# UT-Austin-RPL/FORGE

Measured on AMD Instinct MI355X. Metric: rendered views/sec (5 views, 128^2 px, 64^3 voxel), higher is better.
Workload: dtype f32; 1 GPU; BASELINE configs[1]: FORGE hot path, 1 scene(s)/GPU x 5 input views 256^2 -> 32^3x128 feature grid -> 64^3 render grid -> 5 views x 128^2 rays x 64 samples -> 5 RGB 256^2; HIP rotate, fp32-MFMA implicit-GEMM ResNet-50 trunk / conv1 / ConvGRU (Winograd F(2x2,3x3) x 3 depth taps) / heads / conv_rgb, HIP ray-march (no MIOpen/rocBLAS kernel in the step); eval BN, random-init seeded weights; scenes_per_gpu=1, views_in=5, views_out=5, feature_grid=32, render_grid=64, steps_in_flight=4, launch=hipGraph replay, 4 steps in flight on 4 HIP streams, parallelism=dp1 (scene-sharded, no data-path collective; 4-scalar RCC...

## Files before the change

forge_amd/_lib.py:

```python
import ctypes
import os

import torch

_HERE = os.path.dirname(os.path.abspath(__file__))
LIB_PATH = os.environ.get("FORGE_AMD_LIB") or os.path.join(_HERE, "libforge_hip.so")
_lib = None

_P = ctypes.c_void_p
_I = ctypes.c_int
_F = ctypes.c_float
_D = ctypes.c_double
_LL = ctypes.c_longlong

SIGNATURES = {
    "forge_version": [],
    "forge_last_error": [],
    "forge_rotate_fwd": [_P, _P, _P, _P, _I, _I, _I, _I, _I, _P],
    "forge_rotate_fwd_slots": [_P, _P, _P, _P, _P, _I, _I, _I, _I, _I, _P],
    "forge_rotate_xf_from_poses": [_P, _P, _P, _P, _P, _I, _I, _F, _P],
    "forge_rotate_bwd": [_P, _P, _P, _P, _P, _P, _I, _I, _I, _I, _I, _P],
    "forge_pose_chain_fwd": [_P, _P, _P, _P, _P, _F, _I, _I, _P, _P, _P, _P, _P, _P, _P, _P],
    "forge_colsum": [_P, _I, _P, _P, _LL, _I, _P],
    "forge_adam_small": [_P, _P, _P, _P, _P, _I, _F, _F, _F, _F, _P],
# ... 7 lines not shown
    "forge_resize_bilinear_bwd": [_P, _P, _I, _I, _I, _I, _I, _P],
    "forge_conv_igemm": [_P, _I, _I, _LL, _P, _I, _I, _LL, _P, _P, _P, _P, _F, _P, _P, _P, _P, _P, _P] + [_I] * 10 + [_P] + [_I] * 12 + [_P, _LL, _P, _P],
    "forge_wino_weights": [_P, _P, _I, _I, _I, _I, _P],
    "forge_wino_dy": [_P, _I, _P, _I, _I, _I, _I, _I, _P],
    "forge_wino_wgrad": [_P, _P, _I, _LL, _LL, _P, _I, _LL, _LL, _P, _I, _I, _I, _I, _I, _I, _P],
    "forge_wino_dw": [_P, _P, _I, _I, _I, _P],
    "forge_wino_input": [_P, _I, _LL, _P, _I, _LL, _I, _I, _I, _I, _I, _I, _LL, _P],
    "forge_wino_input_dy": [_P, _I, _P, _P, _I, _I, _I, _I, _I, _P],
    "forge_wino_gemm": [_P, _I, _I, _LL, _LL, _P, _I, _I, _LL, _LL, _P, _P, _I, _I, _I, _I, _I, _I, _I, _P],
    "forge_wino_gemm_half": [_P, _I, _I, _LL, _LL, _P, _I, _I, _LL, _LL, _P, _P, _I, _I, _I, _I, _I, _I, _P],
    "forge_wino_gemm_dn": [_P, _I, _I, _LL, _LL, _P, _I, _I, _LL, _LL, _P, _P, _I, _I, _I, _I, _I, _I, _P],
    "forge_wino_weights_dn": [_P, _P, _I, _I, _P],
    "forge_wino_input_dn4": [_P, _I, _LL, _P, _I, _LL, _I, _I, _I, _I, _I, _I, _LL, _P],
    "forge_wino_weights_dn4": [_P, _P, _I, _I, _P],
    "forge_wino_gemm_dn4": [_P, _I, _I, _LL, _LL, _P, _I, _I, _LL, _LL, _P, _P, _I, _I, _I, _I, _I, _I, _P],
    "forge_wino_input_dn4h": [_P, _I, _LL, _P, _I, _LL, _I, _I, _I, _I, _I, _I, _LL, _P],
    "forge_wino_weights_dn4h": [_P, _P, _I, _I, _P],
    "forge_wino_gemm_dn4h": [_P, _I, _I, _LL, _LL, _P, _I, _I, _LL, _LL, _P, _P, _I, _I, _I, _I, _I, _I, _P],
    "forge_wino_output_dn4h": [_P, _P, _P, _P, _P, _P, _P, _P, _P, _I, _I, _I, _I, _I, _I, _I, _P],
    "forge_wino_output_half": [_P, _P, _LL, _LL, _P, _P, _P, _F, _P, _P, _P, _P, _P, _P, _I, _I, _I, _I, _I, _I, _I, _P],
    "forge_wino_gemm_tile": [_LL, _I, _I],
    "forge_wino_output": [_P, _P, _LL, _LL, _P, _P, _P, _F, _P, _P, _P, _P, _P, _P, _I, _I, _I, _I, _I, _I, _I, _P],
    "forge_conv_igemm_plan": [_LL, _I, _I, _I, _I, _I, _I, _LL, _P, _P],
    "forge_conv_wgrad": [_P, _I, _P, _I, _I, _LL, _P, _I, _I, _LL, _P] + [_I] * 9 + [_P, _I, _P],
    "forge_conv_direct_fwd": [_P, _I, _P, _P, _F, _P, _I] + [_I] * 6 + [_P, _I, _P],
    "forge_conv_direct_dgrad": [_P, _I, _P, _P, _I] + [_I] * 6 + [_P, _I, _P],
    "forge_conv_direct_wgrad": [_P, _I, _P, _I, _P] + [_I] * 6 + [_P, _I, _P],
    "forge_gru_gates_fwd": [_P, _P, _P, _P, _P, _LL, _I, _P],
    "forge_gru_state_fwd": [_P, _P, _P, _P, _LL, _I, _P],
    "forge_gru_state_bwd": [_P, _I, _P, _P, _P, _P, _P, _P, _LL, _I, _P, _LL, _LL, _I, _P],
    "forge_gru_gates_bwd": [_P, _P, _I, _P, _P, _P, _P, _P, _P, _I, _LL, _I, _P, _LL, _LL, _I, _P],
    "forge_bn_ws_doubles": [_I],
    "forge_bn_train_fwd": [_P, _I, _P, _P, _F, _F, _P, _I, _P, _P, _P, _P, _F, _P, _LL, _I, _P, _I, _P, _I, _P],
    "forge_bn_train_bwd": [_P, _I, _P, _I, _P, _P, _P, _P, _F, _P, _I, _P, _P, _P, _LL, _I, _P, _I, _P, _I, _P],
    "forge_bn_sync_stats": [_P, _I, _P, _LL, _I, _I, _P],
    "forge_bn_eval_fwd": [_P, _I, _P, _P, _P, _P, _F, _F, _P, _I, _P, _P, _LL, _I, _P, _I, _P],
    "forge_bn_sync_fwd_apply": [_P, _I, _P, _P, _F, _F, _P, _I, _P, _P, _P, _P, _F, _P, _LL, _LL, _I, _P, _I, _P, _P],
    "forge_bn_sync_bwd_reduce": [_P, _I, _P, _I, _P, _P, _P, _P, _F, _P, _P, _P, _LL, _I, _P, _I, _P],
    "forge_bn_sync_bwd_apply": [_P, _I, _P, _I, _P, _P, _P, _P, _F, _P, _I, _P, _LL, _LL, _I, _P, _I, _P, _I, _P],
    "forge_affine_act_bwd": [_P, _I, _P, _I, _P, _F, _P, _I, _LL, _I, _P],
    "forge_sse_groups_blocks": [],
    "forge_sse_groups_fwd": [_P, _LL, _LL, _LL, _LL, _P, _P] + [_I] * 7 + [_P],
    "forge_sse_groups_bwd": [_P, _LL, _LL, _LL, _LL, _P, _P, _P] + [_I] * 7 + [_P],
    "forge_attention_fwd": [_P, _P, _P, _LL, _P, _I, _I, _I, _I, _P],
    "forge_attention_fwd_lse": [_P, _P, _P, _LL, _P, _P, _I, _I, _I, _I, _P],
    "forge_attention_bwd": [_P, _P, _P, _LL, _P, _P, _P, _P, _P, _P, _P, _I, _I, _I, _I, _P],
# ... 94 lines not shown
```

forge_amd/convops.py:

```python
import collections
import ctypes
import functools
import os
from fractions import Fraction

import torch

from . import _lib, determinism

EPI_BIAS, EPI_AFFINE_ACT, EPI_GRU_GATES, EPI_GRU_OUT = 0, 1, 2, 3


_TAPS_CACHE = {}


def _taps_array(taps):
    key = tuple(tuple(t) for t in taps)
    arr = _TAPS_CACHE.get(key)
    if arr is None:
        flat = [int(v) for t in key for v in t]
        arr = _TAPS_CACHE[key] = (ctypes.c_int * len(flat))(*flat)
    return arr


# ... 154 lines not shown

GRAD_ZEROS = _ZeroArena()


def grad_zeros(shape, device, scratch=False):
    if scratch:
        return torch.zeros(tuple(shape), dtype=torch.float32, device=device)
    return GRAD_ZEROS.zeros(tuple(shape), device)


SPLITK_WS_BYTES = 128 << 20

TILE_NAMES = {"A": "128, 128, 8, 1", "B": "64, 128, 8, 1", "C": "128, 64, 8, 1", "D": "64, 64, 4, 1", "E": "128, 32, 4, 1"}

_PLAN_CACHE = {}


class _State:
    plan_override = None
    winograd = True
    wino_depth_nest = os.environ.get("FORGE_WINO_DEPTH_NEST", "1") != "0"
    wino_depth_nest4 = os.environ.get("FORGE_WINO_DEPTH_NEST4", "1") != "0"
    wino_h4 = os.environ.get("FORGE_WINO_H4", "1") != "0"


STATE = _State()


class force_plan:

    def __init__(self, tile=None, ksplit=None):
        self.val = (tile, ksplit)

    def __enter__(self):
        self.prev = STATE.plan_override
        STATE.plan_override = self.val
        return self

    def __exit__(self, *exc):
        STATE.plan_override = self.prev
        return False


def conv_plan(M, Cout, Cin, ntaps, epilogue, ldo, nphase=1):
    key = (int(M), int(Cout), int(Cin), int(ntaps), int(nphase), int(epilogue), int(ldo) % 4 == 0)
    pl = _PLAN_CACHE.get(key)
    if pl is None:
        tile, ks = ctypes.c_int(0), ctypes.c_int(0)
        _lib.check(_lib.lib().forge_conv_igemm_plan(int(M), int(Cout), int(Cin), int(ntaps), int(nphase), int(epilogue), int(ldo), SPLITK_WS_BYTES,
                                                    ctypes.byref(tile), ctypes.byref(ks)), "forge_conv_igemm_plan")
        pl = _PLAN_CACHE[key] = (chr(tile.value), ks.value)
    ov = STATE.plan_override
    if ov is not None and pl[0] != "N":
        tile = ov[0] or pl[0]
        ks = ov[1] if ov[1] is not None else (pl[1] if ov[0] is None else 1)
        can_split = nphase == 1 and epilogue in (EPI_BIAS, EPI_AFFINE_ACT) and Cout % 4 == 0 and ldo % 4 == 0
        if ks > 1 and not (can_split and ks * M * Cout * 4 <= SPLITK_WS_BYTES and ks <= (ntaps // nphase) * (Cin // 32)):
            ks = 1
        return tile, ks
    return pl


MAX_OPERAND_BYTES = (1 << 31) - 1


@_lib.on_tensor_device
def conv_igemm(in1, C1, ld1, in2, C2, ld2, wp, bias, scale, shift, slope, residual, aux_h, aux_z, out, out2,
               grid, in_grid, Cout, ldo, taps, out_grid=None, istride=1, ostride=1, phase=(0, 0, 0), epilogue=EPI_BIAS,
               bs1=0, bs2=0, lift=0, out3=None, stats=None):
    n, D, H, W = grid
    Di, Hi, Wi = in_grid
    Do, Ho, Wo = out_grid if out_grid is not None else (D, H, W)
    if wp.shape != (len(taps), Cout, C1 + C2):
        raise ValueError("packed weight %s does not match taps=%d Cout=%d Cin=%d" % (tuple(wp.shape), len(taps), Cout, C1 + C2))
    in_rows, out_rows = Di * Hi * Wi, Do * Ho * Wo
    b1, b2 = (int(bs1) or in_rows), (int(bs2) or in_rows)
    span = lambda k, br, ld: ((k - 1) * br + in_rows) * ld * 4
    limit = MAX_OPERAND_BYTES
    nc = n
    while nc > 1 and (span(nc, b1, ld1) > limit or (in2 is not None and span(nc, b2, ld2) > limit)):
        nc = (nc + 1) // 2
    L, st, arr = _lib.lib(), _lib.current_stream(), _taps_array(taps)
    nphase = 1
    if tuple(phase) == (-1, -1, -1):
        nphase = 8 if Do == 2 * D else 4

    def off(t, floats):
        return None if t is None else ctypes.c_void_p(t.data_ptr() + 4 * floats)
    gate_w = Cout // 2 if epilogue == EPI_GRU_GATES else Cout
    for s0 in range(0, n, nc):
        k = min(nc, n - s0)
        orow = s0 * out_rows
        tile, ksplit = conv_plan(k * D * H * W, Cout, C1 + C2, len(taps), epilogue, ldo, nphase)
        if stats is not None and (ksplit > 1 or nc < n):
            raise RuntimeError("forge_amd: conv_igemm output statistics need an un-chunked launch without split-K (use conv_stats_buffer)")
        ws = torch.empty(ksplit * k * D * H * W * Cout, dtype=torch.float32, device=out.device) if ksplit > 1 else None
        o_ld = gate_w if epilogue == EPI_GRU_GATES else ldo
        _lib.check(L.forge_conv_igemm(
            off(in1, s0 * b1 * ld1), C1, ld1, int(bs1), off(in2, s0 * b2 * ld2), C2, ld2, int(bs2), _lib.ptr(wp), _lib.ptr(bias), _lib.ptr(scale),
            _lib.ptr(shift), float(slope), off(residual, orow * (Cout if (lift or epilogue in (EPI_GRU_GATES, EPI_GRU_OUT)) else ldo)),
            off(aux_h, orow * gate_w), off(aux_z, orow * Cout),
            off(out, orow * (Cout if lift else o_ld)), off(out2, orow * o_ld), off(out3, orow * o_ld), k, D, H, W, istride, Di, Hi, Wi, Cout, ldo,
            arr, len(taps), ostride, phase[0], phase[1], phase[2], Do, Ho, Wo, epilogue, int(lift), 0 if tile == "N" else ord(tile), ksplit,
            _lib.ptr(ws), 0 if ws is None else ws.numel() * 4, _lib.ptr(stats), st),
            "forge_conv_igemm")
# ... 226 lines not shown
        Mm = torch.empty(P, R, Cout, dtype=torch.float32, device=device)
    if not (Mm.is_contiguous() and Mm.dtype == torch.float32 and Mm.numel() >= P * R * Cout):
        raise ValueError("point-product buffer %s %s%s cannot hold %d x %d x %d float32" % (
            tuple(Mm.shape), Mm.dtype, "" if Mm.is_contiguous() else " (not contiguous)", P, R, Cout))
    if Mm.shape != (P, R, Cout):
        Mm = Mm.as_strided((P, R, Cout), (R * Cout, Cout, 1))
    return Mm


@_lib.on_tensor_device
def wino_form_gemm(form, V1, C1, V2, C2, U, Mm, n, D, Ht, Wt, Cout, view=0, views=1):
    R = n * D * Ht * Wt
    vol = int(D * Ht * Wt * form.rows)
    nest = form.kloops is not None
    kd = 3 if nest else U.shape[1]
    if U.shape != form.ushape(kd, Cout, C1 + C2) or (kd not in (1, 3)) or (nest and not U.is_contiguous()):
        raise ValueError("%s weight %s does not match Cout=%d Cin=%d" % ("depth-nest" if nest else "transformed", tuple(U.shape), Cout, C1 + C2))
    if form.rows != 1 and (V1.shape[1] != n * views * vol or (V2 is not None and V2.shape[1] != n * vol)):
        raise ValueError("depth-nest operands %s / %s are not %s's %d (x %d views) rows per point" % (
            tuple(V1.shape), None if V2 is None else tuple(V2.shape), form.input, n * vol, views))
    Mm = _point_products(Mm, form.P, R, Cout, V1.device)
    tile = (ord(wino_gemm_tile(R, Cout, C1 + C2)),) if form.tile else ()
    p1 = ctypes.c_void_p(V1.data_ptr() + 4 * view * vol * C1)
    _lib.check(getattr(_lib.lib(), form.gemm)(p1, C1, C1, views * vol if views > 1 else 0, V1.shape[1] * C1, _lib.ptr(V2), C2, C2, 0,
                                              0 if V2 is None else V2.shape[1] * C2, _lib.ptr(U), _lib.ptr(Mm), n, D, Ht, Wt, Cout, kd,
                                              *tile, _lib.current_stream()), form.gemm)
    return Mm


def wino_gemm(V1, C1, V2, C2, U, Mm, n, D, Ht, Wt, Cout, view=0, views=1, half=None):
    if U.dim() == 5:
        form = "dn"
    else:
        if half is None:
            half = WINO_FORMS["half"].applies(n * D * Ht * Wt, D, Ht, Wt, Cout, C1 + C2)
        form = "half" if half else "points"
    return wino_form_gemm(WINO_FORMS[form], V1, C1, V2, C2, U, Mm, n, D, Ht, Wt, Cout, view=view, views=views)


def wino_gemm_tile(R, Cout, Cin):
    ov = STATE.plan_override
    if ov is not None and ov[0]:
        return ov[0]
    return chr(_lib.lib().forge_wino_gemm_tile(int(R), int(Cout), int(Cin)))


@_lib.on_tensor_device
def wino_output(Mm, bias, scale, shift, slope, residual, aux_h, aux_z, out, out2, out3, n, D, H, W, Cout, ldo, epilogue, Mm2=None, view=0, views=1):
    P = Mm.shape[0] if Mm.dim() == 3 else 0
# ... 401 lines not shown
```

forge_amd/csrc/conv_igemm.hip:

```cpp
#include "common.h"
#include <cmath>
#include <type_traits>

namespace forge {

enum ConvEpilogue : int {
    EPI_BIAS = 0,
    EPI_AFFINE_ACT = 1,
    EPI_GRU_GATES = 2,
    EPI_GRU_OUT = 3,
};

constexpr int MAX_TAPS = 64;

struct ConvArgs {
    const float* in1; const float* in2;
    int C1, C2, ld1, ld2;
    long long bs1r, bs2r;
    long long span1, span2;
    const float* wp;
    const float* bias;
    const float* scale; const float* shift; float slope;
    const float* aux_h; const float* aux_z;
    float* out; float* out2; float* out3;
    int n, D, H, W;
    int is, Di, Hi, Wi;
    const float* residual; int ldr;
    int Cout, ldo;
    int ntaps;
    int os, pz, py, px, Do, Ho, Wo;
    int nphase, tpp;
    int epi;
    int lift;
    int nbat;
    long long pt1, pt2, ptw, pto;
    float* ws; int ksplit;
    double* stats;
    signed char tap[MAX_TAPS][4];
};

constexpr int BK = 32, NTHREADS = 512;
constexpr int RS_STAGES = 2;

#ifdef FORGE_CONV_TIMING
__device__ long long g_conv_stamp[8192 * 4];
#define FORGE_STAMP(k) do { if (threadIdx.x == 0 && blockIdx.x < 8192) g_conv_stamp[blockIdx.x * 4 + (k)] = wall_clock64(); } while (0)
extern "C" int forge_debug_conv_stamps(long long* host, int n) {
    return (int)hipMemcpyFromSymbol(host, HIP_SYMBOL(g_conv_stamp), (size_t)n * 4 * sizeof(long long));
}
#else
#define FORGE_STAMP(k) do { } while (0)
#endif

__device__ __forceinline__ int lds_off(int row, int chunk) {
    return row * BK + ((chunk ^ ((row >> 1) & 7)) << 2);
}

struct LanePos { int wm, wn, half, l31; };

struct ReadA {
// ... 71 lines not shown
        store(1, [&](int r) { return acc[1][0][0][r] - acc[0][0][0][r]; });
        FORGE_STAMP(3);
    }
}

template <int BM, int BN, int NW, int MT = 1, int RS = 0>
__global__ __launch_bounds__(NW * 64) void conv_igemm_kernel(const ConvArgs a) {
    constexpr int NP = RS ? 4 : 1;
    constexpr int WM = BM / (32 * MT), WN = NW / WM;
    constexpr int NT = BN / (32 * WN);
    static_assert(NT >= 1 && WM * WN == NW && NT * 32 * WN == BN && WM * 32 * MT == BM, "unsupported tile");
    constexpr int A_FLOATS = BM * BK, B_FLOATS = BN * BK;
    constexpr int RPP = NW * 8;
    constexpr int ACH = BM / RPP, BCH = BN / RPP;
    static_assert(ACH >= 1 && BCH >= 1, "tile too small for the workgroup");
    extern __shared__ __attribute__((aligned(16))) float smem[];

    FORGE_STAMP(0);
    const int tid = threadIdx.x, lane = tid & 63, wave = tid >> 6;
    const int wm = wave / WN, wn = wave % WN;
    const long long M = (long long)a.n * a.D * a.H * a.W;
    const int ntile_n = (a.Cout + BN - 1) / BN;
    const unsigned bid_all = xcd_remap(blockIdx.x, gridDim.x);
    const int ks = (int)(bid_all % (unsigned)a.ksplit);
    unsigned bid = bid_all / (unsigned)a.ksplit;
    int phase = 0;
    if (a.nphase > 1) {
        phase = (int)(bid % (unsigned)a.nphase);
        bid /= (unsigned)a.nphase;
    }
    const int pz = a.nphase > 1 ? (a.nphase == 8 ? (phase >> 2) & 1 : 0) : a.pz;
    const int py = a.nphase > 1 ? (phase >> 1) & 1 : a.py, px = a.nphase > 1 ? phase & 1 : a.px;
    const int t_lo = phase * a.tpp;
    constexpr int PLANES = RS == 2 ? 2 : RS == 3 ? 4 : 1;
    long long pb = 0;
    if (a.nbat > 1) {
        const unsigned tiles = (PLANES > 1 ? (unsigned)(M / (PLANES * BM)) : (unsigned)((M + BM - 1) / BM)) * (unsigned)ntile_n;
        pb = bid / tiles;
        bid -= (unsigned)pb * tiles;
    }
    float* const outp = a.out + pb * a.pto;
    const long long m0 = [&]() -> long long {
        if constexpr (PLANES > 1) {
            const unsigned tpl = (unsigned)(a.H * a.W) / BM;
            const unsigned ti = bid / ntile_n, grp = ti / tpl;
            return (long long)((unsigned)PLANES * grp * tpl + (ti - grp * tpl)) * BM;
        } else {
            return (long long)(bid / ntile_n) * BM;
        }
    }();
    const int n0 = (bid % ntile_n) * BN;
    const int Cin = a.C1 + a.C2;
    const int kchunks = Cin / BK;
    const int nsteps_all = a.tpp * kchunks;
    const int s_begin = (int)((long long)ks * nsteps_all / a.ksplit), s_end = (int)((long long)(ks + 1) * nsteps_all / a.ksplit);
    const int nsteps = s_end - s_begin;

    forge_v4i32 w1 = make_rsrc_words(a.in1 + pb * a.pt1, a.span1), w2 = make_rsrc_words(a.in2 ? a.in2 + pb * a.pt2 : a.in1, a.in2 ? a.span2 : 0),
                ww = make_rsrc_words(a.wp + pb * a.ptw, (long long)a.ntaps * a.Cout * Cin * 4);
    const unsigned lds_wave = lds_addr(smem) + (unsigned)__builtin_amdgcn_readfirstlane(wave) * 1024u;
    const int cp = tid & 7;
    int ar[ACH], az[ACH], ay[ACH], ax[ACH], an[ACH], asrc[ACH];
    bool aval[ACH];
#pragma unroll
    for (int j = 0; j < ACH; ++j) {
        ar[j] = (tid >> 3) + RPP * j;
        const long long vl = m0 + ar[j];
        aval[j] = vl < M;
        unsigned v = aval[j] ? (unsigned)vl : 0u;
        unsigned q = v / (unsigned)a.W;
        ax[j] = (int)(v - q * (unsigned)a.W) * a.is; v = q;
        q = v / (unsigned)a.H;
        ay[j] = (int)(v - q * (unsigned)a.H) * a.is; v = q;
        q = v / (unsigned)a.D;
        az[j] = (int)(v - q * (unsigned)a.D) * a.is;
        an[j] = (int)q;
        asrc[j] = (cp ^ ((ar[j] >> 1) & 7)) << 2;
    }
    int br[BCH]; unsigned boff[BCH];
#pragma unroll
    for (int j = 0; j < BCH; ++j) {
        br[j] = (tid >> 3) + RPP * j;
        const int bsrc = (cp ^ ((br[j] >> 1) & 7)) << 2;
        boff[j] = (n0 + br[j]) < a.Cout ? (unsigned)(((n0 + br[j]) * Cin + bsrc) * 4) : OOB;
    }

    constexpr bool KC_OUTER = (BM == 128 && BN == 128);
    static_assert(!RS || (!KC_OUTER && MT == 1), "the row-stage form exists on the tap-outer tiles");
    __shared__ int sdelta[KC_OUTER ? 2 * MAX_TAPS : 1];
    unsigned long long vmask[KC_OUTER ? ACH : 1];
    unsigned base1[KC_OUTER ? ACH : 1], base2[KC_OUTER ? ACH : 1];
    if constexpr (KC_OUTER) {
#pragma unroll
        for (int j = 0; j < ACH; ++j) {
            const int sp = (az[j] * a.Hi + ay[j]) * a.Wi + ax[j];
            base1[j] = (unsigned)(((an[j] * (int)a.bs1r + sp) * a.ld1 + asrc[j]) * 4);
            base2[j] = (unsigned)(((an[j] * (int)a.bs2r + sp) * a.ld2 + asrc[j]) * 4);
            vmask[j] = 0ull;
        }
        for (int tt = 0; tt < a.ntaps; ++tt) {
            const int dz = a.tap[tt][0], dy = a.tap[tt][1], dx = a.tap[tt][2];
#pragma unroll
            for (int j = 0; j < ACH; ++j) {
                const int zi = az[j] + dz, yi = ay[j] + dy, xi = ax[j] + dx;
                const bool ok = aval[j] && (unsigned)zi < (unsigned)a.Di && (unsigned)yi < (unsigned)a.Hi && (unsigned)xi < (unsigned)a.Wi;
                vmask[j] |= (unsigned long long)ok << tt;
            }
        }
        if (tid < a.ntaps) {
            const int d = (a.tap[tid][0] * a.Hi + a.tap[tid][1]) * a.Wi + a.tap[tid][2];
            sdelta[tid] = d * a.ld1 * 4;
            sdelta[MAX_TAPS + tid] = d * a.ld2 * 4;
        }
        __syncthreads();
    }
    unsigned eoff[ACH], eoff2[ACH];
    auto prep_tap = [&](int t) {
        if constexpr (KC_OUTER) {
            const unsigned d1 = (unsigned)sdelta[t], d2 = (unsigned)sdelta[MAX_TAPS + t];
#pragma unroll
            for (int j = 0; j < ACH; ++j) {
                const bool ok = (vmask[j] >> t) & 1ull;
                eoff[j] = ok ? base1[j] + d1 : OOB;
                eoff2[j] = ok ? base2[j] + d2 : OOB;
            }
        } else {
            const int dz = a.tap[t][0], dy = a.tap[t][1], dx = a.tap[t][2];
#pragma unroll
            for (int j = 0; j < ACH; ++j) {
                const int zi = az[j] + dz, yi = ay[j] + dy, xi = ax[j] + dx;
                const bool ok = aval[j] && (unsigned)zi < (unsigned)a.Di && (unsigned)yi < (unsigned)a.Hi && (unsigned)xi < (unsigned)a.Wi;
                const int sp = (zi * a.Hi + yi) * a.Wi + xi;
                eoff[j] = ok ? (unsigned)(((an[j] * (int)a.bs1r + sp) * a.ld1 + asrc[j]) * 4) : OOB;
                eoff2[j] = ok ? (unsigned)(((an[j] * (int)a.bs2r + sp) * a.ld2 + asrc[j]) * 4) : OOB;
            }
        }
    };
    auto issue_step = [&](int t, int kc, int buf) {
        const int c0 = kc * BK;
        const unsigned stage = lds_wave + (unsigned)buf * (unsigned)((A_FLOATS + B_FLOATS) * 4);
        if (c0 < a.C1) {
#pragma unroll
            for (int j = 0; j < ACH; ++j) lds_dma16(w1, eoff[j] + (unsigned)(c0 * 4), stage + (unsigned)(j * NW * 1024));
        } else {
#pragma unroll
            for (int j = 0; j < ACH; ++j) lds_dma16(w2, eoff2[j] + (unsigned)((c0 - a.C1) * 4), stage + (unsigned)(j * NW * 1024));
        }
        const unsigned wbase = (unsigned)((t * a.Cout * Cin + c0) * 4);
#pragma unroll
        for (int j = 0; j < BCH; ++j) lds_dma16(ww, boff[j] + wbase, stage + (unsigned)(A_FLOATS * 4 + j * NW * 1024));
    };
    constexpr int NACC = RS == 3 ? 4 : RS ? 3 : 1;
    f32x16 accs[NACC][MT][NT];
#pragma unroll
    for (int q = 0; q < NACC; ++q)
#pragma unroll
        for (int i = 0; i < MT; ++i)
#pragma unroll
            for (int j = 0; j < NT; ++j)
#pragma unroll
                for (int r = 0; r < 16; ++r) accs[q][i][j][r] = 0.f;
    f32x16 (&acc)[MT][NT] = accs[0];

    const int half = lane >> 5, l31 = lane & 31;
    int kc, t;
    if constexpr (KC_OUTER) { kc = s_begin / a.tpp; t = s_begin - kc * a.tpp; }
    else { t = s_begin / kchunks; kc = s_begin - t * kchunks; }
    t += t_lo;
    auto advance = [&]() {
        if constexpr (KC_OUTER) {
            if (++t == t_lo + a.tpp) { t = t_lo; ++kc; }
            prep_tap(t);
        } else {
            if (++kc == kchunks) { kc = 0; ++t; prep_tap(t); }
        }
    };
    if constexpr (!RS) {
        prep_tap(t);
        issue_step(t, kc, 0);
        lds_dma_wait();
        __syncthreads();
        FORGE_STAMP(1);
    }
    const LanePos lp{wm, wn, half, l31};
    [[maybe_unused]] const unsigned HW = (unsigned)(a.H * a.W);
    [[maybe_unused]] const int col0 = n0 + wn * (BN / WN);
    if constexpr (!RS) {
    int buf = 0;
#pragma unroll
    for (int q = 0; q < NP; ++q) {
        for (int s = 0; s < nsteps; ++s) {
            const float* sa = smem + buf * (A_FLOATS + B_FLOATS);
            const float* sb = sa + A_FLOATS;
            if (s + 1 < nsteps) {
                advance();
                issue_step(t, kc, buf ^ 1);
            }
#pragma unroll
            for (int g = 0; g < 4; ++g) mfma_group<BN, WN, MT, NT>(lp, accs[q], sa, sb, g, ReadA{});
            lds_dma_wait();
            __syncthreads();
            buf ^= 1;
// ... 134 lines not shown
                }
            } else if (q == 3) {
#pragma unroll
                for (int r = 0; r < 16; ++r) {
                    const float S = accs[2][0][0][r] + accs[3][0][0][r], Dl = accs[2][0][0][r] - accs[3][0][0][r];
                    accs[2][0][0][r] = fmaf(4.f, S, accs[0][0][0][r]);
                    accs[3][0][0][r] = fmaf(2.f, Dl, accs[1][0][0][r]);
                    accs[0][0][0][r] = accs[0][0][0][r] + S;
                    accs[1][0][0][r] = fmaf(8.f, Dl, accs[1][0][0][r]);
                }
                store(1, accs[3][0][0]);
                store(2, accs[2][0][0]);
            } else if (q == 4) {
                store(0, accs[0][0][0]);
            }
        }
        FORGE_STAMP(2);
        store(3, accs[1][0][0]);
        FORGE_STAMP(3);
    }
    if constexpr (RS != 0) return;

    FORGE_STAMP(2);
    const int Ch = a.Cout / 2;
    const bool remap = (a.os != 1) || (a.Do != a.D) || (a.Ho != a.H) || (a.Wo != a.W);
    long long* s_row = reinterpret_cast<long long*>(smem);
    if (a.ksplit == 1 && tid < BM) {
        const long long m = m0 + tid;
        long long o = -1;
        if (m < M) {
            if (a.lift > 0) {
                const unsigned HW = (unsigned)(a.H * a.W), nn = (unsigned)m / HW, hw = (unsigned)m - nn * HW;
                o = ((long long)nn * a.lift * HW + hw) * (a.Cout / a.lift);
            } else if (remap) {
                unsigned q = (unsigned)m, t2 = q / (unsigned)a.W;
                const int x = (int)(q - t2 * (unsigned)a.W); q = t2; t2 = q / (unsigned)a.H;
                const int y = (int)(q - t2 * (unsigned)a.H); q = t2; t2 = q / (unsigned)a.D;
                const int z = (int)(q - t2 * (unsigned)a.D);
                o = (((long long)t2 * a.Do + (z * a.os + pz)) * a.Ho + (y * a.os + py)) * a.Wo + (x * a.os + px);
            } else {
                o = m;
            }
        }
        s_row[tid] = o;
    }
    __syncthreads();
// ... 454 lines not shown
                ++rounds;
            }
            const double traffic_us = ((double)M * K * 4.0 * ntn + (double)Cout * K * 4.0 + (double)M * Cout * 4.0) / 4.0e6;
            if (us < traffic_us) us = traffic_us;
            us += (double)(rounds + 1) * t.ov * sqrt((double)t.bm * t.bn / 16384.0);
            if (k > 1) us += 3.0 + (double)(k + 1) * M * Cout * 4.0 / 2.0e6;
            if (us < best_us) { best_us = us; best = ConvPlan{t.id, k}; }
        }
    }
    return best;
}

template <int RS>
static int launch_point_form(const ConvArgs& a, int planes, size_t lds, const char* entry, hipStream_t st) {
    const long long M = (long long)a.n * a.D * a.H * a.W;
    const long long grid = ((M + 64 * planes - 1) / (64 * planes)) * ((a.Cout + 127) / 128) * a.nbat;
    FORGE_REQUIRE(grid < (1ll << 31), FORGE_ESHAPE, "%s: grid too large", entry);
    FORGE_REQUIRE(RS != 1 || M * a.ldo * 4 < (1ll << 31), FORGE_ESHAPE, "%s: an output plane spans >= 2 GiB (32-bit buffer offsets); split the batch", entry);
    FORGE_SET_MAX_LDS_ONCE((conv_igemm_kernel<64, 128, 8, 1, RS>), lds);
    hipLaunchKernelGGL((conv_igemm_kernel<64, 128, 8, 1, RS>), dim3((unsigned)grid), dim3(8 * 64), lds, st, a);
    return 0;
}

static int launch_conv_tile(const ConvArgs& a, char tile, hipStream_t st, int row_stage = 0) {
    const long long M = (long long)a.n * a.D * a.H * a.W;
    auto nblk = [&](int bm, int bn) { return ((M + bm - 1) / bm) * ((a.Cout + bn - 1) / bn); };
    if (row_stage == 1) { const size_t lds = RS_STAGES * (64 * BK + 128 * BK) * sizeof(float); return launch_point_form<1>(a, 1, lds, "forge_wino_gemm_half", st); }
    if (row_stage == 2) { const size_t lds = RS_STAGES * (2 * 64 * BK + 128 * BK) * sizeof(float); return launch_point_form<2>(a, 2, lds, "forge_wino_gemm_dn", st); }
    if (row_stage == 3) { const size_t lds = RS_STAGES * (64 * BK + 128 * BK) * sizeof(float); return launch_point_form<3>(a, 4, lds, "forge_wino_gemm_dn4", st); }
#define FORGE_LAUNCH_CONV(BMv, BNv, NWv)                                                                                   \
    do {                                                                                                                   \
        const long long grid = nblk(BMv, BNv) * a.ksplit * a.nphase * a.nbat;                                              \
        FORGE_REQUIRE(grid < (1ll << 31), FORGE_ESHAPE, "forge_conv_igemm: grid too large");                                \
        const size_t lds = 2 * (BMv * BK + BNv * BK) * sizeof(float);                                                      \
        FORGE_SET_MAX_LDS_ONCE((conv_igemm_kernel<BMv, BNv, NWv>), lds);                                                   \
        hipLaunchKernelGGL((conv_igemm_kernel<BMv, BNv, NWv>), dim3((unsigned)grid), dim3(NWv * 64), lds, st, a);          \
    } while (0)
    switch (tile) {
        case 'A': FORGE_LAUNCH_CONV(128, 128, 8); break;
        case 'B': FORGE_LAUNCH_CONV(64, 128, 8); break;
        case 'C': FORGE_LAUNCH_CONV(128, 64, 8); break;
        case 'E': FORGE_LAUNCH_CONV(128, 32, 4); break;
        default: FORGE_LAUNCH_CONV(64, 64, 4); break;
    }
#undef FORGE_LAUNCH_CONV
    return 0;
}

}

using namespace forge;

extern "C" int forge_conv_igemm_plan(long long M, int Cout, int Cin, int ntaps, int nphase, int epilogue, int ldo, long long splitk_ws_bytes,
                                     int* tile, int* ksplit) {
    FORGE_REQUIRE(tile && ksplit && M > 0 && Cout > 0 && Cin > 0 && ntaps > 0 && (nphase == 1 || nphase == 4 || nphase == 8) && ntaps % nphase == 0,
                  FORGE_EINVAL, "forge_conv_igemm_plan: bad argument");
    if (Cout <= 16) { *tile = 'N'; *ksplit = 1; return 0; }
    const ConvPlan pl = plan_conv(M * nphase, Cout, Cin, ntaps / nphase,
                                  nphase == 1 && splitk_ws_bytes > 0 && (epilogue == EPI_BIAS || epilogue == EPI_AFFINE_ACT) && Cout % 4 == 0 && ldo % 4 == 0,
                                  splitk_ws_bytes);
    *tile = pl.tile; *ksplit = pl.ksplit;
    return 0;
}

extern "C" int forge_conv_igemm(const float* in1, int C1, int ld1, long long bs1, const float* in2, int C2, int ld2, long long bs2,
                                const float* wp,
                                const float* bias, const float* scale, const float* shift, float slope, const float* residual,
                                const float* aux_h, const float* aux_z, float* out, float* out2, float* out3,
                                int n, int D, int H, int W, int is, int Di, int Hi, int Wi, int Cout, int ldo,
                                const int* taps, int ntaps, int os, int pz, int py, int px, int Do, int Ho, int Wo,
                                int epilogue, int lift, int tile, int ksplit, float* splitk_ws, long long splitk_ws_bytes, double* stats,
                                forge_stream_t stream) {
    FORGE_REQUIRE(in1 && wp && out && taps, FORGE_EINVAL, "forge_conv_igemm: null pointer argument");
    FORGE_REQUIRE(stats == nullptr || (epilogue == EPI_BIAS && ksplit <= 1 && Cout > 16 && !(pz < 0) && lift == 0), FORGE_EINVAL,
                  "forge_conv_igemm: output statistics need the plain bias epilogue of the wide kernel without split-K, phases or lift");
    FORGE_REQUIRE(n > 0 && D > 0 && H > 0 && W > 0 && Cout > 0 && ntaps > 0 && ntaps <= MAX_TAPS, FORGE_EINVAL,
                  "forge_conv_igemm: bad dims n=%d D=%d H=%d W=%d Cout=%d ntaps=%d", n, D, H, W, Cout, ntaps);
    const int kstep = Cout <= 16 ? 16 : 32;
    FORGE_REQUIRE(C1 > 0 && C1 % kstep == 0 && C2 >= 0 && C2 % kstep == 0, FORGE_ESHAPE,
                  "forge_conv_igemm: C1=%d / C2=%d must be multiples of the K-step %d (16 for Cout <= 16, else 32)", C1, C2, kstep);
    FORGE_REQUIRE((C2 == 0) == (in2 == nullptr), FORGE_EINVAL, "forge_conv_igemm: in2/C2 mismatch");
    FORGE_REQUIRE(epilogue >= 0 && epilogue <= 3, FORGE_EINVAL, "forge_conv_igemm: unknown epilogue %d", epilogue);
    FORGE_REQUIRE(epilogue != EPI_AFFINE_ACT || (scale && shift), FORGE_EINVAL, "forge_conv_igemm: affine epilogue needs scale/shift");
    FORGE_REQUIRE(epilogue != EPI_GRU_GATES || (aux_h && out2 && Cout % 2 == 0), FORGE_EINVAL, "forge_conv_igemm: GRU gate epilogue needs aux_h, out2");
    FORGE_REQUIRE(epilogue != EPI_GRU_OUT || (aux_h && aux_z), FORGE_EINVAL, "forge_conv_igemm: GRU out epilogue needs aux_h, aux_z");
    FORGE_REQUIRE(os >= 1 && Do > 0 && Ho > 0 && Wo > 0, FORGE_EINVAL, "forge_conv_igemm: bad output mapping");
    FORGE_REQUIRE(is >= 1 && Di > 0 && Hi > 0 && Wi > 0, FORGE_EINVAL, "forge_conv_igemm: bad input mapping");
    FORGE_REQUIRE(lift == 0 || (lift > 0 && epilogue == EPI_AFFINE_ACT && Cout % lift == 0 && D == 1 && os == 1 && Cout > 64), FORGE_EINVAL,
                  "forge_conv_igemm: lift needs the affine epilogue on a 2-D (D=1) conv with Cout %% lift == 0 and Cout > 64");
    FORGE_REQUIRE(ld1 >= C1 && ld1 % 4 == 0 && (C2 == 0 || (ld2 >= C2 && ld2 % 4 == 0)) && ldo >= 1, FORGE_EINVAL,
                  "forge_conv_igemm: row strides must cover the channels and keep 16-byte alignment");
    ConvArgs a;
    a.in1 = in1; a.in2 = in2; a.C1 = C1; a.C2 = C2; a.ld1 = ld1; a.ld2 = ld2;
    a.bs1r = bs1 > 0 ? bs1 : (long long)Di * Hi * Wi; a.bs2r = bs2 > 0 ? bs2 : (long long)Di * Hi * Wi;
    a.span1 = ((long long)(n - 1) * a.bs1r + (long long)Di * Hi * Wi) * ld1 * 4;
    a.span2 = in2 ? ((long long)(n - 1) * a.bs2r + (long long)Di * Hi * Wi) * ld2 * 4 : 0;
    FORGE_REQUIRE(a.span1 < (1ll << 31) && a.span2 < (1ll << 31) && (long long)ntaps * Cout * (C1 + C2) * 4 < (1ll << 31), FORGE_ESHAPE,
                  "forge_conv_igemm: an operand spans >= 2 GiB (32-bit buffer offsets); split the batch");
    a.is = is; a.Di = Di; a.Hi = Hi; a.Wi = Wi; a.residual = residual;
    a.ldr = (lift > 0 || epilogue == EPI_GRU_GATES || epilogue == EPI_GRU_OUT) ? Cout : ldo;
    a.lift = lift; a.ws = nullptr; a.ksplit = 1; a.stats = stats;
    a.wp = wp; a.bias = bias; a.scale = scale; a.shift = shift; a.slope = slope;
    a.aux_h = aux_h; a.aux_z = aux_z; a.out = out; a.out2 = out2; a.out3 = out3; a.n = n; a.D = D; a.H = H; a.W = W; a.Cout = Cout; a.ldo = ldo;
    a.ntaps = ntaps; a.os = os; a.pz = pz; a.py = py; a.px = px; a.Do = Do; a.Ho = Ho; a.Wo = Wo; a.epi = epilogue;
    a.nphase = 1; a.tpp = ntaps; a.nbat = 1; a.pt1 = a.pt2 = a.ptw = a.pto = 0;
    if (pz < 0) {
        FORGE_REQUIRE(os == 2 && py < 0 && px < 0 && Ho == 2 * H && Wo == 2 * W && (Do == 2 * D || Do == D), FORGE_EINVAL,
                      "forge_conv_igemm: merged phases (pz = py = px = -1) need os = 2 and a doubled output grid");
        a.nphase = Do == 2 * D ? 8 : 4;
        FORGE_REQUIRE(ntaps % a.nphase == 0, FORGE_EINVAL, "forge_conv_igemm: merged phases need ntaps %% %d == 0", a.nphase);
        a.tpp = ntaps / a.nphase;
        a.pz = a.py = a.px = 0;
    }
    for (int k = 0; k < 3 * ntaps; ++k)
        FORGE_REQUIRE(taps[k] >= -128 && taps[k] <= 127, FORGE_EINVAL, "forge_conv_igemm: tap %d component %d = %d outside [-128, 127]", k / 3, k % 3, taps[k]);
    for (int t = 0; t < MAX_TAPS; ++t) {
        for (int k = 0; k < 3; ++k) a.tap[t][k] = (signed char)(t < ntaps ? taps[t * 3 + k] : 0);
        a.tap[t][3] = 0;
    }
    const long long M = (long long)n * D * H * W;
    FORGE_REQUIRE(M < (1ll << 31), FORGE_ESHAPE, "forge_conv_igemm: more than 2^31 GEMM rows; split the batch");
    FORGE_REQUIRE(out3 == nullptr || epilogue == EPI_GRU_GATES || epilogue == EPI_GRU_OUT, FORGE_EINVAL, "forge_conv_igemm: out3 is a GRU-epilogue output");
    hipStream_t st = (hipStream_t)stream;
    if (Cout <= 16) {
// ... 121 lines not shown
```

include/forge_hip.h:

```cpp
#ifndef FORGE_HIP_H
#define FORGE_HIP_H

#ifdef __cplusplus
extern "C" {
#endif

typedef void* forge_stream_t;

#define FORGE_EINVAL (-1)
#define FORGE_ESHAPE (-2)

int forge_version(void);
const char* forge_last_error(void);

int forge_rotate_fwd(const float* vox, const float* xf, const int* mode, float* out,
                     int n, int C, int D, int H, int W, forge_stream_t stream);

int forge_rotate_fwd_slots(const float* vox, const float* xf, const int* mode, const int* dst_slot, float* out,
                           int n, int C, int D, int H, int W, forge_stream_t stream);

int forge_rotate_xf_from_poses(const float* poses, float* xf, int* mode, int* slot, const float* dist, int B, int t, float half_extent,
                               forge_stream_t stream);

int forge_pose_chain_fwd(const float* rot, const float* trans, const float* can_pose, const float* can_extr, const float* K, float half_extent,
// ... 16 lines not shown
                       const float* K, long long k0, long long k1, long long k2, float* cam16, float* origin, int V, forge_stream_t stream);

long long forge_render_bwd_ws_bytes(int V, int C, int Hr, int Wr, int S, int want_cam);
int forge_render_bwd(const float* feat, const float* dens, const float* cam, const int* view2vol,
                     const float* g_feat, const float* g_opac, const float* g_depth,
                     float* dfeat, float* ddens, float* dcam,
                     int V, int nvol, int C, int D, int H, int W, int Hr, int Wr, int S,
                     float zmin, float zmax, float hx, float hy, float hz,
                     void* ws, long long ws_bytes, forge_stream_t stream);

int forge_resize_bilinear_fwd(const float* in, float* out, int P, int Hi, int Wi, int Ho, int Wo, forge_stream_t stream);
int forge_resize_bilinear_bwd(const float* g, float* din, int P, int Hi, int Wi, int Ho, int Wo, forge_stream_t stream);

int forge_conv_igemm(const float* in1, int C1, int ld1, long long bs1, const float* in2, int C2, int ld2, long long bs2,
                     const float* wp,
                     const float* bias, const float* scale, const float* shift, float slope, const float* residual,
                     const float* aux_h, const float* aux_z, float* out, float* out2, float* out3,
                     int n, int D, int H, int W, int is, int Di, int Hi, int Wi, int Cout, int ldo,
                     const int* taps, int ntaps, int os, int pz, int py, int px, int Do, int Ho, int Wo,
                     int epilogue, int lift, int tile, int ksplit, float* splitk_ws, long long splitk_ws_bytes, double* stats, forge_stream_t stream);

int forge_conv_igemm_plan(long long M, int Cout, int Cin, int ntaps, int nphase, int epilogue, int ldo, long long splitk_ws_bytes,
                          int* tile, int* ksplit);

int forge_wino_weights(const float* wp, float* U, int Cout, int Cin, int kd, int transpose, forge_stream_t stream);
int forge_wino_dy(const float* dy, int ldy, float* dM, int n, int D, int H, int W, int Cout, forge_stream_t stream);
int forge_wino_wgrad(const float* dMm, const float* V1, int C1, long long bs1, long long pt1, const float* V2, int C2, long long bs2,
                     long long pt2, float* dU, int n, int D, int Ht, int Wt, int Cout, int kd, forge_stream_t stream);
int forge_wino_dw(const float* dU, float* dw, int Cout, int Cin, int kd, forge_stream_t stream);
int forge_wino_input(const float* in, int ld, long long bs, float* V, int ldv, long long ptv, int n, int D, int H, int W, int C,
                     int nsum , long long sum_stride,
                     forge_stream_t stream);
int forge_wino_input_dy(const float* dy, int ld, float* V, float* dM, int n, int D, int H, int W, int C, forge_stream_t stream);
int forge_wino_gemm(const float* V1, int C1, int ld1, long long bs1, long long pt1, const float* V2, int C2, int ld2, long long bs2,
                    long long pt2, const float* U, float* Mm, int n, int D, int Ht, int Wt, int Cout, int kd, int tile ,
                    forge_stream_t stream);
int forge_wino_gemm_half(const float* V1, int C1, int ld1, long long bs1, long long pt1, const float* V2, int C2, int ld2, long long bs2,
                         long long pt2, const float* U, float* Mm8, int n, int D, int Ht, int Wt, int Cout, int kd, forge_stream_t stream);
int forge_wino_output_half(const float* Mm8, const float* Mm2_8 , long long bs2, long long pt2, const float* bias, const float* scale,
                           const float* shift, float slope, const float* residual, const float* aux_h, const float* aux_z, float* out, float* out2, float* out3,
                           int n, int D, int H, int W, int Cout, int ldo, int epilogue, forge_stream_t stream);
int forge_wino_gemm_dn(const float* V1, int C1, int ld1, long long bs1, long long pt1, const float* V2, int C2, int ld2, long long bs2,
                       long long pt2, const float* Ud, float* Mm, int n, int D, int Ht, int Wt, int Cout, int kd, forge_stream_t stream);
int forge_wino_weights_dn(const float* wp, float* Ud, int Cout, int Cin, forge_stream_t stream);
int forge_wino_input_dn4(const float* in, int ld, long long bs, float* V6, int ldv, long long ptv, int n, int D, int H, int W, int C,
                         int nsum, long long sum_stride, forge_stream_t stream);
// ... 174 lines not shown
```

Before: 989.5 views/s.

## Add direct register-to-global conv epilogue, flat 1x1 row indexing, early weight prefetch

Adds a fast epilogue path to the implicit-GEMM conv kernel that writes bias/affine/residual/leaky results straight from MFMA accumulators to global memory with buffer stores. This skips the LDS-staged row-remap epilogue for simple same-grid, non-split, non-stat cases. It also treats pointwise 1x1 convs as flat rows, which avoids per-row div/mod coordinate decoding. The first weight tile DMA is now issued before the A-side address prep, and the k-split arithmetic is skipped when unused. The direct stores are strided per lane and less coalesced than the staged epilogue, which could hurt bandwidth on wide outputs.

```diff
diff --git a/forge_amd/_lib.py b/forge_amd/_lib.py
--- a/forge_amd/_lib.py
+++ b/forge_amd/_lib.py
@@ -53,6 +53,8 @@
     "forge_wino_gemm_tile": [_LL, _I, _I],
     "forge_wino_output": [_P, _P, _LL, _LL, _P, _P, _P, _F, _P, _P, _P, _P, _P, _P, _I, _I, _I, _I, _I, _I, _I, _P],
     "forge_conv_igemm_plan": [_LL, _I, _I, _I, _I, _I, _I, _LL, _P, _P],
+    "forge_conv_igemm_epilogue": [_LL] + [_I] * 11 + [_P],
+    "forge_conv_fast_epilogue": [_I],
     "forge_conv_wgrad": [_P, _I, _P, _I, _I, _LL, _P, _I, _I, _LL, _P] + [_I] * 9 + [_P, _I, _P],
     "forge_conv_direct_fwd": [_P, _I, _P, _P, _F, _P, _I] + [_I] * 6 + [_P, _I, _P],
     "forge_conv_direct_dgrad": [_P, _I, _P, _P, _I] + [_I] * 6 + [_P, _I, _P],
diff --git a/forge_amd/convops.py b/forge_amd/convops.py
--- a/forge_amd/convops.py
+++ b/forge_amd/convops.py
@@ -200,6 +200,7 @@
     wino_depth_nest = os.environ.get("FORGE_WINO_DEPTH_NEST", "1") != "0"
     wino_depth_nest4 = os.environ.get("FORGE_WINO_DEPTH_NEST4", "1") != "0"
     wino_h4 = os.environ.get("FORGE_WINO_H4", "1") != "0"
+    conv_fast_epilogue = os.environ.get("FORGE_CONV_FAST_EPILOGUE", "1") != "0"
 
 
 STATE = _State()
@@ -218,6 +219,27 @@
     def __exit__(self, *exc):
         STATE.plan_override = self.prev
         return False
+
+
+_pushed_fast_epilogue = None
+
+
+def _conv_lib():
+    global _pushed_fast_epilogue
+    L = _lib.lib()
+    want = bool(STATE.conv_fast_epilogue)
+    if want is not _pushed_fast_epilogue:
+        L.forge_conv_fast_epilogue(int(want))
+        _pushed_fast_epilogue = want
+    return L
+
+
+def conv_epilogue_is_direct(M, Cout, ldo, ldr=0, residual=False, ostride=1, same_grid=True, nphase=1, lift=0, ksplit=1, stats=False, epilogue=EPI_BIAS):
+    fast = ctypes.c_int(0)
+    _lib.check(_conv_lib().forge_conv_igemm_epilogue(int(M), int(Cout), int(ldo), int(ldr), int(bool(residual)), int(ostride), int(bool(same_grid)),
+                                                     int(nphase), int(lift), int(ksplit), int(bool(stats)), int(epilogue), ctypes.byref(fast)),
+               "forge_conv_igemm_epilogue")
+    return bool(fast.value)
 
 
 def conv_plan(M, Cout, Cin, ntaps, epilogue, ldo, nphase=1):
@@ -258,7 +280,7 @@
     nc = n
     while nc > 1 and (span(nc, b1, ld1) > limit or (in2 is not None and span(nc, b2, ld2) > limit)):
         nc = (nc + 1) // 2
-    L, st, arr = _lib.lib(), _lib.current_stream(), _taps_array(taps)
+    L, st, arr = _conv_lib(), _lib.current_stream(), _taps_array(taps)
     nphase = 1
     if tuple(phase) == (-1, -1, -1):
         nphase = 8 if Do == 2 * D else 4
@@ -531,9 +553,9 @@
     Mm = _point_products(Mm, form.P, R, Cout, V1.device)
     tile = (ord(wino_gemm_tile(R, Cout, C1 + C2)),) if form.tile else ()
     p1 = ctypes.c_void_p(V1.data_ptr() + 4 * view * vol * C1)
-    _lib.check(getattr(_lib.lib(), form.gemm)(p1, C1, C1, views * vol if views > 1 else 0, V1.shape[1] * C1, _lib.ptr(V2), C2, C2, 0,
-                                              0 if V2 is None else V2.shape[1] * C2, _lib.ptr(U), _lib.ptr(Mm), n, D, Ht, Wt, Cout, kd,
-                                              *tile, _lib.current_stream()), form.gemm)
+    _lib.check(getattr(_conv_lib(), form.gemm)(p1, C1, C1, views * vol if views > 1 else 0, V1.shape[1] * C1, _lib.ptr(V2), C2, C2, 0,
+                                               0 if V2 is None else V2.shape[1] * C2, _lib.ptr(U), _lib.ptr(Mm), n, D, Ht, Wt, Cout, kd,
+                                               *tile, _lib.current_stream()), form.gemm)
     return Mm
 
 
diff --git a/forge_amd/csrc/conv_igemm.hip b/forge_amd/csrc/conv_igemm.hip
--- a/forge_amd/csrc/conv_igemm.hip
+++ b/forge_amd/csrc/conv_igemm.hip
@@ -36,6 +36,8 @@
     long long pt1, pt2, ptw, pto;
     float* ws; int ksplit;
     double* stats;
+    int flat_rows;
+    int fast_epi;
     signed char tap[MAX_TAPS][4];
 };
 
@@ -153,8 +155,9 @@
     const long long M = (long long)a.n * a.D * a.H * a.W;
     const int ntile_n = (a.Cout + BN - 1) / BN;
     const unsigned bid_all = xcd_remap(blockIdx.x, gridDim.x);
-    const int ks = (int)(bid_all % (unsigned)a.ksplit);
-    unsigned bid = bid_all / (unsigned)a.ksplit;
+    int ks = 0;
+    unsigned bid = bid_all;
+    if (!RS && a.ksplit > 1) { ks = (int)(bid_all % (unsigned)a.ksplit); bid = bid_all / (unsigned)a.ksplit; }
     int phase = 0;
     if (a.nphase > 1) {
         phase = (int)(bid % (unsigned)a.nphase);
@@ -184,13 +187,38 @@
     const int Cin = a.C1 + a.C2;
     const int kchunks = Cin / BK;
     const int nsteps_all = a.tpp * kchunks;
-    const int s_begin = (int)((long long)ks * nsteps_all / a.ksplit), s_end = (int)((long long)(ks + 1) * nsteps_all / a.ksplit);
+    int s_begin = 0, s_end = nsteps_all;
+    if (!RS && a.ksplit > 1) {
+        s_begin = (int)((unsigned)ks * (unsigned)nsteps_all / (unsigned)a.ksplit);
+        s_end = (int)((unsigned)(ks + 1) * (unsigned)nsteps_all / (unsigned)a.ksplit);
+    }
     const int nsteps = s_end - s_begin;
 
     forge_v4i32 w1 = make_rsrc_words(a.in1 + pb * a.pt1, a.span1), w2 = make_rsrc_words(a.in2 ? a.in2 + pb * a.pt2 : a.in1, a.in2 ? a.span2 : 0),
                 ww = make_rsrc_words(a.wp + pb * a.ptw, (long long)a.ntaps * a.Cout * Cin * 4);
     const unsigned lds_wave = lds_addr(smem) + (unsigned)__builtin_amdgcn_readfirstlane(wave) * 1024u;
     const int cp = tid & 7;
+    int br[BCH]; unsigned boff[BCH];
+#pragma unroll
+    for (int j = 0; j < BCH; ++j) {
+        br[j] = (tid >> 3) + RPP * j;
+        const int bsrc = (cp ^ ((br[j] >> 1) & 7)) << 2;
+        boff[j] = (n0 + br[j]) < a.Cout ? (unsigned)(((n0 + br[j]) * Cin + bsrc) * 4) : OOB;
+    }
+    constexpr bool KC_OUTER = (BM == 128 && BN == 128);
+    int kc, t;
+    if constexpr (KC_OUTER) { kc = s_begin / a.tpp; t = s_begin - kc * a.tpp; }
+    else { t = s_begin / kchunks; kc = s_begin - t * kchunks; }
+    t += t_lo;
+    auto issue_b = [&](int t, int kc, int buf) {
+        const unsigned stage = lds_wave + (unsigned)buf * (unsigned)((A_FLOATS + B_FLOATS) * 4);
+        const unsigned wbase = (unsigned)((t * a.Cout * Cin + kc * BK) * 4);
+#pragma unroll
+        for (int j = 0; j < BCH; ++j) lds_dma16(ww, boff[j] + wbase, stage + (unsigned)(A_FLOATS * 4 + j * NW * 1024));
+    };
+    if constexpr (!RS) issue_b(t, kc, 0);
+    const bool flat = !RS && a.flat_rows;
+    const int Wi_ = flat ? (int)M : a.Wi;
     int ar[ACH], az[ACH], ay[ACH], ax[ACH], an[ACH], asrc[ACH];
     bool aval[ACH];
 #pragma unroll
@@ -199,24 +227,20 @@
         const long long vl = m0 + ar[j];
         aval[j] = vl < M;
         unsigned v = aval[j] ? (unsigned)vl : 0u;
-        unsigned q = v / (unsigned)a.W;
-        ax[j] = (int)(v - q * (unsigned)a.W) * a.is; v = q;
-        q = v / (unsigned)a.H;
-        ay[j] = (int)(v - q * (unsigned)a.H) * a.is; v = q;
-        q = v / (unsigned)a.D;
-        az[j] = (int)(v - q * (unsigned)a.D) * a.is;
-        an[j] = (int)q;
+        if (flat) {
+            ax[j] = (int)v; ay[j] = az[j] = an[j] = 0;
+        } else {
+            unsigned q = v / (unsigned)a.W;
+            ax[j] = (int)(v - q * (unsigned)a.W) * a.is; v = q;
+            q = v / (unsigned)a.H;
+            ay[j] = (int)(v - q * (unsigned)a.H) * a.is; v = q;
+            q = v / (unsigned)a.D;
+            az[j] = (int)(v - q * (unsigned)a.D) * a.is;
+            an[j] = (int)q;
+        }
         asrc[j] = (cp ^ ((ar[j] >> 1) & 7)) << 2;
     }
-    int br[BCH]; unsigned boff[BCH];
-#pragma unroll
-    for (int j = 0; j < BCH; ++j) {
-        br[j] = (tid >> 3) + RPP * j;
-        const int bsrc = (cp ^ ((br[j] >> 1) & 7)) << 2;
-        boff[j] = (n0 + br[j]) < a.Cout ? (unsigned)(((n0 + br[j]) * Cin + bsrc) * 4) : OOB;
-    }
-
-    constexpr bool KC_OUTER = (BM == 128 && BN == 128);
+
     static_assert(!RS || (!KC_OUTER && MT == 1), "the row-stage form exists on the tap-outer tiles");
     __shared__ int sdelta[KC_OUTER ? 2 * MAX_TAPS : 1];
     unsigned long long vmask[KC_OUTER ? ACH : 1];
@@ -234,7 +258,7 @@
 #pragma unroll
             for (int j = 0; j < ACH; ++j) {
                 const int zi = az[j] + dz, yi = ay[j] + dy, xi = ax[j] + dx;
-                const bool ok = aval[j] && (unsigned)zi < (unsigned)a.Di && (unsigned)yi < (unsigned)a.Hi && (unsigned)xi < (unsigned)a.Wi;
+                const bool ok = aval[j] && (unsigned)zi < (unsigned)a.Di && (unsigned)yi < (unsigned)a.Hi && (unsigned)xi < (unsigned)Wi_;
                 vmask[j] |= (unsigned long long)ok << tt;
             }
         }
@@ -260,14 +284,14 @@
 #pragma unroll
             for (int j = 0; j < ACH; ++j) {
                 const int zi = az[j] + dz, yi = ay[j] + dy, xi = ax[j] + dx;
-                const bool ok = aval[j] && (unsigned)zi < (unsigned)a.Di && (unsigned)yi < (unsigned)a.Hi && (unsigned)xi < (unsigned)a.Wi;
+                const bool ok = aval[j] && (unsigned)zi < (unsigned)a.Di && (unsigned)yi < (unsigned)a.Hi && (unsigned)xi < (unsigned)Wi_;
                 const int sp = (zi * a.Hi + yi) * a.Wi + xi;
                 eoff[j] = ok ? (unsigned)(((an[j] * (int)a.bs1r + sp) * a.ld1 + asrc[j]) * 4) : OOB;
                 eoff2[j] = ok ? (unsigned)(((an[j] * (int)a.bs2r + sp) * a.ld2 + asrc[j]) * 4) : OOB;
             }
         }
     };
-    auto issue_step = [&](int t, int kc, int buf) {
+    auto issue_a = [&](int t, int kc, int buf) {
         const int c0 = kc * BK;
         const unsigned stage = lds_wave + (unsigned)buf * (unsigned)((A_FLOATS + B_FLOATS) * 4);
         if (c0 < a.C1) {
@@ -277,10 +301,8 @@
 #pragma unroll
             for (int j = 0; j < ACH; ++j) lds_dma16(w2, eoff2[j] + (unsigned)((c0 - a.C1) * 4), stage + (unsigned)(j * NW * 1024));
         }
-        const unsigned wbase = (unsigned)((t * a.Cout * Cin + c0) * 4);
-#pragma unroll
-        for (int j = 0; j < BCH; ++j) lds_dma16(ww, boff[j] + wbase, stage + (unsigned)(A_FLOATS * 4 + j * NW * 1024));
     };
+    auto issue_step = [&](int t, int kc, int buf) { issue_a(t, kc, buf); issue_b(t, kc, buf); };
     constexpr int NACC = RS == 3 ? 4 : RS ? 3 : 1;
     f32x16 accs[NACC][MT][NT];
 #pragma unroll
@@ -294,10 +316,6 @@
     f32x16 (&acc)[MT][NT] = accs[0];
 
     const int half = lane >> 5, l31 = lane & 31;
-    int kc, t;
-    if constexpr (KC_OUTER) { kc = s_begin / a.tpp; t = s_begin - kc * a.tpp; }
-    else { t = s_begin / kchunks; kc = s_begin - t * kchunks; }
-    t += t_lo;
     auto advance = [&]() {
         if constexpr (KC_OUTER) {
             if (++t == t_lo + a.tpp) { t = t_lo; ++kc; }
@@ -308,7 +326,7 @@
     };
     if constexpr (!RS) {
         prep_tap(t);
-        issue_step(t, kc, 0);
+        issue_a(t, kc, 0);
         lds_dma_wait();
         __syncthreads();
         FORGE_STAMP(1);
@@ -489,6 +507,57 @@
     if constexpr (RS != 0) return;
 
     FORGE_STAMP(2);
+    if (a.fast_epi) {
+        const __amdgpu_buffer_rsrc_t ro = make_rsrc(outp, ((M - 1) * a.ldo + a.Cout) * 4);
+        const unsigned row0 = (unsigned)m0 + (unsigned)(wm * (32 * MT) + 4 * half);
+        const unsigned ldo4 = (unsigned)a.ldo * 4u;
+        auto direct = [&](auto EPI_TAG, auto RES_TAG) {
+            constexpr int EPI = decltype(EPI_TAG)::value;
+            constexpr bool RES = decltype(RES_TAG)::value;
+            float res[RES ? NT : 1][MT][16];
+            if constexpr (RES) {
+                const __amdgpu_buffer_rsrc_t rr = make_rsrc(a.residual, ((M - 1) * a.ldr + a.Cout) * 4);
+                const unsigned ldr4 = (unsigned)a.ldr * 4u;
+#pragma unroll
+                for (int j = 0; j < NT; ++j) {
+                    const int col = col0 + j * 32 + l31;
+                    const unsigned rb = col < a.Cout ? (row0 * (unsigned)a.ldr + (unsigned)col) * 4u : OOB;
+#pragma unroll
+                    for (int i = 0; i < MT; ++i)
+#pragma unroll
+                        for (int r = 0; r < 16; ++r)
+                            res[j][i][r] = __uint_as_float(__builtin_amdgcn_raw_buffer_load_b32(rr, (int)(rb + (unsigned)(i * 32 + (r & 3) + 8 * (r >> 2)) * ldr4), 0, 0));
+                }
+            }
+#pragma unroll
+            for (int j = 0; j < NT; ++j) {
+                const int col = col0 + j * 32 + l31;
+                const bool cok = col < a.Cout;
+                const int colc = cok ? col : 0;
+                const float bias = a.bias ? a.bias[colc] : 0.f;
+                float sc = 1.f, sh = 0.f;
+                if (EPI == EPI_AFFINE_ACT && a.scale) { sc = a.scale[colc]; sh = a.shift[colc]; }
+                const unsigned vb = cok ? (row0 * (unsigned)a.ldo + (unsigned)col) * 4u : OOB;
+#pragma unroll
+                for (int i = 0; i < MT; ++i)
+#pragma unroll
+                    for (int r = 0; r < 16; ++r) {
+                        float v = acc[i][j][r] + bias;
+                        if constexpr (EPI == EPI_AFFINE_ACT) {
+                            v = fmaf(v, sc, sh);
+                            if constexpr (RES) v += res[j][i][r];
+                            v = v > 0.f ? v : v * a.slope;
+                        }
+                        __builtin_amdgcn_raw_buffer_store_b32(__float_as_uint(v), ro, (int)(vb + (unsigned)(i * 32 + (r & 3) + 8 * (r >> 2)) * ldo4), 0, 0);
+                    }
+            }
+        };
+        if (a.epi == EPI_BIAS) direct(std::integral_constant<int, EPI_BIAS>{}, std::false_type{});
+        else if (a.residual) direct(std::integral_constant<int, EPI_AFFINE_ACT>{}, std::true_type{});
+        else direct(std::integral_constant<int, EPI_AFFINE_ACT>{}, std::false_type{});
+        FORGE_STAMP(3);
+        return;
+    }
     const int Ch = a.Cout / 2;
     const bool remap = (a.os != 1) || (a.Do != a.D) || (a.Ho != a.H) || (a.Wo != a.W);
     long long* s_row = reinterpret_cast<long long*>(smem);
@@ -989,8 +1058,25 @@
     return 0;
 }
 
-static int launch_conv_tile(const ConvArgs& a, char tile, hipStream_t st, int row_stage = 0) {
+static bool g_conv_fast_epilogue = true;
+
+static bool conv_fast_epilogue_applies(long long M, int Cout, int ldo, int ldr, bool residual, int os, bool same_grid, int nphase, int lift, int ksplit,
+                                       bool stats, int epi) {
+    if (ksplit != 1 || os != 1 || !same_grid || nphase != 1 || lift != 0 || stats) return false;
+    if (epi != EPI_BIAS && epi != EPI_AFFINE_ACT) return false;
+    if (M < 1 || Cout < 1 || ldo < Cout || ldo >= (1 << 22) || ((M - 1) * ldo + Cout) * 4 >= (1ll << 31)) return false;
+    if (residual && epi == EPI_AFFINE_ACT && (ldr < Cout || ldr >= (1 << 22) || ((M - 1) * ldr + Cout) * 4 >= (1ll << 31))) return false;
+    return true;
+}
+
+static int launch_conv_tile(const ConvArgs& args, char tile, hipStream_t st, int row_stage = 0) {
+    ConvArgs a = args;
     const long long M = (long long)a.n * a.D * a.H * a.W;
+    a.flat_rows = row_stage == 0 && a.ntaps == 1 && a.nphase == 1 && a.tap[0][0] == 0 && a.tap[0][1] == 0 && a.tap[0][2] == 0 && a.is == 1 && a.Di == a.D &&
+                  a.Hi == a.H && a.Wi == a.W && a.bs1r == (long long)a.D * a.H * a.W && (a.in2 == nullptr || a.bs2r == a.bs1r);
+    a.fast_epi = row_stage == 0 && g_conv_fast_epilogue && (a.nbat == 1 || a.epi == EPI_BIAS) &&
+                 conv_fast_epilogue_applies(M, a.Cout, a.ldo, a.ldr, a.residual != nullptr, a.os, a.Do == a.D && a.Ho == a.H && a.Wo == a.W, a.nphase, a.lift,
+                                            a.ksplit, a.stats != nullptr, a.epi);
     auto nblk = [&](int bm, int bn) { return ((M + bm - 1) / bm) * ((a.Cout + bn - 1) / bn); };
     if (row_stage == 1) { const size_t lds = RS_STAGES * (64 * BK + 128 * BK) * sizeof(float); return launch_point_form<1>(a, 1, lds, "forge_wino_gemm_half", st); }
     if (row_stage == 2) { const size_t lds = RS_STAGES * (2 * 64 * BK + 128 * BK) * sizeof(float); return launch_point_form<2>(a, 2, lds, "forge_wino_gemm_dn", st); }
@@ -1027,6 +1113,21 @@
                                   nphase == 1 && splitk_ws_bytes > 0 && (epilogue == EPI_BIAS || epilogue == EPI_AFFINE_ACT) && Cout % 4 == 0 && ldo % 4 == 0,
                                   splitk_ws_bytes);
     *tile = pl.tile; *ksplit = pl.ksplit;
+    return 0;
+}
+
+extern "C" int forge_conv_fast_epilogue(int on) {
+    const int prev = g_conv_fast_epilogue;
+    if (on >= 0) g_conv_fast_epilogue = on != 0;
+    return prev;
+}
+
+extern "C" int forge_conv_igemm_epilogue(long long M, int Cout, int ldo, int ldr, int has_residual, int os, int same_grid, int nphase, int lift, int ksplit,
+                                         int has_stats, int epilogue, int* fast) {
+    FORGE_REQUIRE(fast && M > 0 && Cout > 0 && ldo > 0 && os >= 1 && nphase >= 1 && lift >= 0 && ksplit >= 1 && epilogue >= 0 && epilogue <= 3, FORGE_EINVAL,
+                  "forge_conv_igemm_epilogue: bad argument");
+    *fast = Cout > 16 && g_conv_fast_epilogue &&
+            conv_fast_epilogue_applies(M, Cout, ldo, ldr, has_residual != 0, os, same_grid != 0, nphase, lift, ksplit, has_stats != 0, epilogue);
     return 0;
 }
 
@@ -1066,7 +1167,7 @@
                   "forge_conv_igemm: an operand spans >= 2 GiB (32-bit buffer offsets); split the batch");
     a.is = is; a.Di = Di; a.Hi = Hi; a.Wi = Wi; a.residual = residual;
     a.ldr = (lift > 0 || epilogue == EPI_GRU_GATES || epilogue == EPI_GRU_OUT) ? Cout : ldo;
-    a.lift = lift; a.ws = nullptr; a.ksplit = 1; a.stats = stats;
+    a.lift = lift; a.ws = nullptr; a.ksplit = 1; a.stats = stats; a.flat_rows = a.fast_epi = 0;
     a.wp = wp; a.bias = bias; a.scale = scale; a.shift = shift; a.slope = slope;
     a.aux_h = aux_h; a.aux_z = aux_z; a.out = out; a.out2 = out2; a.out3 = out3; a.n = n; a.D = D; a.H = H; a.W = W; a.Cout = Cout; a.ldo = ldo;
     a.ntaps = ntaps; a.os = os; a.pz = pz; a.py = py; a.px = px; a.Do = Do; a.Ho = Ho; a.Wo = Wo; a.epi = epilogue;
diff --git a/include/forge_hip.h b/include/forge_hip.h
--- a/include/forge_hip.h
+++ b/include/forge_hip.h
@@ -62,6 +62,10 @@
 
 int forge_conv_igemm_plan(long long M, int Cout, int Cin, int ntaps, int nphase, int epilogue, int ldo, long long splitk_ws_bytes,
                           int* tile, int* ksplit);
+
+int forge_conv_igemm_epilogue(long long M, int Cout, int ldo, int ldr, int has_residual, int os, int same_grid, int nphase, int lift, int ksplit,
+                              int has_stats, int epilogue, int* fast);
+int forge_conv_fast_epilogue(int on);
 
 int forge_wino_weights(const float* wp, float* U, int Cout, int Cin, int kd, int transpose, forge_stream_t stream);
 int forge_wino_dy(const float* dy, int ldy, float* dM, int n, int D, int H, int W, int Cout, forge_stream_t stream);
```

After: 1026 views/s, median of 6. +3.7%, better.
